# tspooner/rsrl

Hardware: AMD Instinct MI355X
Metric: env-steps/sec (whole node), MountainCar Q-learning Fourier-5 (higher is better)
Workload: dtype f32

## Files before the change

rsrl_amd/_build.py:

```python
import os
import shutil
import subprocess

HERE = os.path.dirname(os.path.abspath(__file__))
CSRC = os.path.join(HERE, "csrc")
LIB_DIR = os.path.join(HERE, "lib")
LIB_PATH = os.path.join(LIB_DIR, "librsrl_hip.so")

HIPCC_FLAGS = ["--offload-arch=gfx950", "-O3", "-std=c++17", "-ffp-contract=off", "-fno-slp-vectorize", "-fPIC",
               "-shared", "-fno-gpu-rdc", "-Wall", "-Wno-unused-function"]


PER_SOURCE_FLAGS = {name: ["-mllvm", "-amdgpu-sched-strategy=" + os.environ.get("RSRL_SCHED_STRATEGY", "max-ilp")]
                    for name in ("train_reg_d0a.hip", "train_reg_d0b.hip", "train_reg_d1.hip", "train_reg_d2.hip")}


ABI_UNITS = ("abi_ctx.hip", "abi_trait.hip", "abi_weights.hip", "abi_train.hip", "abi_group.hip", "kernels_util.hip", "launch_shared.hip")
for _u in ABI_UNITS:
    PER_SOURCE_FLAGS[_u] = ["-mllvm", "-disable-promote-alloca-to-lds"]


def hipcc():
    for cand in (os.environ.get("HIPCC"), shutil.which("hipcc"), "/opt/rocm/bin/hipcc"):
        if cand and os.path.exists(cand):
            return cand
    raise RuntimeError("hipcc not found (need ROCm >= 7.0)")


def sources():
    return [os.path.join(CSRC, f) for f in sorted(os.listdir(CSRC)) if f.endswith(".hip")]


def deps():
    inc = os.path.join(os.path.dirname(HERE), "include", "rsrl_hip.h")
    return [os.path.join(CSRC, f) for f in os.listdir(CSRC)] + [inc, os.path.abspath(__file__), os.path.join(HERE, "_asmfilter.py")]


STAMP_PATH = LIB_PATH + ".sha256"


def source_digest(extra_flags=()):
    import hashlib
    h = hashlib.sha256()
    files = sorted(os.path.join(CSRC, f) for f in os.listdir(CSRC)) + [os.path.join(os.path.dirname(HERE), "include", "rsrl_hip.h")]
    for f in files:
        h.update(os.path.basename(f).encode() + b"\0")
        h.update(open(f, "rb").read())
    h.update(repr((HIPCC_FLAGS, sorted(PER_SOURCE_FLAGS.items()), list(extra_flags), nop_filter_enabled(), NOP_FILTER_SOURCES)).encode())
    h.update(open(os.path.join(HERE, "_asmfilter.py"), "rb").read())
    h.update(hipcc_version().encode())
    return h.hexdigest()


_HIPCC_VERSION = None


def hipcc_version():
    global _HIPCC_VERSION
    if _HIPCC_VERSION is None:
        try:
            _HIPCC_VERSION = subprocess.run([hipcc(), "--version"], capture_output=True, text=True, timeout=60).stdout.strip()
        except Exception:
            _HIPCC_VERSION = ""
    return _HIPCC_VERSION


def is_stale():
# ... 139 lines not shown
```

rsrl_amd/csrc/abi_ctx.hip:

```cpp
#include "ctx.hpp"

thread_local std::string g_last_error;

int fail(int code, const char* fmt, ...) {
    char buf[512];
    va_list ap; va_start(ap, fmt); vsnprintf(buf, sizeof(buf), fmt, ap); va_end(ap);
    g_last_error = buf;
    if (code == RSRL_HIP_EHIP || code == RSRL_HIP_ENOMEM) (void)hipGetLastError();
    return code;
}

static Switches read_switches() {
    Switches sw;
    sw.no_graph = getenv("RSRL_NO_GRAPH") != nullptr;
    sw.no_persist = getenv("RSRL_NO_PERSIST") != nullptr;
    sw.no_trait_defer = getenv("RSRL_NO_TRAIT_DEFER") != nullptr;
    sw.k1_feature_major = getenv("RSRL_K1_FEATURE_MAJOR") != nullptr;
    if (const char* e = getenv("RSRL_K1_QUAD")) sw.k1_quad = e[0] != '0' ? 1 : 0;
    if (const char* e = getenv("RSRL_SPARSE_CHUNK")) { const int v = atoi(e); sw.sparse_chunk = v > 0 && v < 16 ? 16 : v; }
    if (const char* e = getenv("RSRL_PEER_TIMEOUT_MS")) sw.peer_timeout_ms = atol(e);
    if (const char* e = getenv("RSRL_WAVE_PK")) sw.no_wave_pk = e[0] == '0';
    return sw;
}
bool no_coalesce_switch() { return getenv("RSRL_NO_COALESCE") != nullptr; }

static AgentFamily classify(const rsrl_hip_config& cfg, size_t w_elems) {
    using F = AgentFamily;
    const bool fourier = cfg.basis == RSRL_FOURIER, tile = cfg.basis == RSRL_TILE_CODING;
    const bool wave = is_wave(cfg), reg = is_reg_fourier(cfg);
    const int al = cfg.algo;
    if (cfg.domain == RSRL_HIV_TREATMENT) return F::Hiv;
    if (is_ac(al)) return F::AcReg;
    if (is_tdac(al)) return F::TdAcReg;
    if (is_reinforce(al)) return F::ReinforceReg;
    if (is_lstd(al)) return F::LstdReg;
    if (is_tdac_lstd(al)) return F::TdAcLstdReg;
    if (cfg.weight_mode == RSRL_W_SHARED) return fourier ? F::SharedDense : (is_sparse_lambda(cfg) ? F::SharedSparseLambda : F::SharedTile);
    if (wave && is_wave_aux_algo(al)) return F::WaveAux;
    if (is_pred(al)) return tile ? F::TdTile : (reg ? F::TdReg : F::TdGeneric);
    if (al == RSRL_Q_SIGMA) return wave ? F::WaveQSigma : (reg ? F::QSigmaReg : F::QSigmaGeneric);
    if (al == RSRL_GREEDY_GQ) return reg ? F::GqReg : F::GqGeneric;
    if (is_lambda(al)) return tile ? F::LambdaTile : (wave ? F::WaveLambda : (reg ? F::LambdaReg : F::LambdaGeneric));
    if (wave) return F::WaveControl;
    if (reg) return cfg.steps_per_launch == 1 && (uint64_t)w_elems * 4ull < (1ull << 32) ? F::RegStep : F::RegFused;
    return F::Generic;
}
static const char* train_kernel_name(const rsrl_hip_ctx* c) {
    switch (c->family) {
    case AgentFamily::SharedDense: return "k_shared_step";
    case AgentFamily::SharedTile: return "k_shared_ca";
    case AgentFamily::SharedSparseLambda: return "k_sparse_trace_scatter";
    case AgentFamily::WaveAux: return "k_wave_aux";
    case AgentFamily::TdTile: return "k_td_tile";
    case AgentFamily::TdGeneric: return "k_td_mem";
    case AgentFamily::TdReg: return "k_train_td";
    case AgentFamily::WaveQSigma: return "k_wave_qsigma";
    case AgentFamily::QSigmaReg: case AgentFamily::QSigmaGeneric: return "k_train_qsigma";
    case AgentFamily::GqReg: return "k_train_gq";
    case AgentFamily::GqGeneric: return "k_train_gq_mem";
    case AgentFamily::LambdaTile: return "k_lambda_tile";
    case AgentFamily::WaveLambda: return "k_wave_lambda";
    case AgentFamily::LambdaGeneric: return "k_train_lambda_mem";
    case AgentFamily::LambdaReg: return "k_train_lambda";
    case AgentFamily::WaveControl: return c->cfg.weight_dtype == RSRL_W_BF16 && !c->sw.no_wave_pk ? "k_train_wave_pk" : "k_train_wave";
    case AgentFamily::RegStep: return c->w_ls != 1 ? (c->k1_quad ? "k_step_reg_q4" : "k_step_reg_lm") : "k_step_reg";
    case AgentFamily::RegFused: return "k_train_reg";
    case AgentFamily::Generic: return "k_train_mem";
    case AgentFamily::Hiv: return "k_hiv_train";
    case AgentFamily::AcReg: return "k_train_ac";
    case AgentFamily::TdAcReg: return "k_train_tdac";
    case AgentFamily::ReinforceReg: return "k_train_reinforce";
    case AgentFamily::LstdReg: return "k_train_lstd";
    case AgentFamily::TdAcLstdReg: return "k_train_tdac_lstd";
    }
// ... 183 lines not shown
    }
    if (shared && wave) return fail(RSRL_HIP_EINVAL, "shared weights are not available for the order-7 wave family yet");
    if (shared && !tile && !reg)
        return fail(RSRL_HIP_EINVAL, "shared weights need a register-family Fourier order (MountainCar 1-5, CartPole/Acrobot 1) or tile coding");
    if (!f32 && !wave) return fail(RSRL_HIP_EINVAL, "bf16 weights are available for Fourier order 7 on CartPole / Acrobot only");
    if (!model_supported(cfg))
        return fail(RSRL_HIP_EINVAL, "basis %d (order %d / %d tilings) on domain %d has no kernel yet", cfg.basis, cfg.order, cfg.n_tilings, cfg.domain);
    if (is_pred(al)) {
        if (!per_env) return fail(RSRL_HIP_EINVAL, "the prediction agents (TD, TDLambda) need per-learner weights on a Fourier basis or on tile coding");
        if (cfg.policy != RSRL_RANDOM) return fail(RSRL_HIP_EINVAL, "prediction agents have no Q function: the behaviour policy must be RSRL_RANDOM");
    }
    if (al == RSRL_GREEDY_GQ && !per_env) return fail(RSRL_HIP_EINVAL, "GreedyGQ needs per-learner weights");
    if (al == RSRL_Q_SIGMA && !per_env) return fail(RSRL_HIP_EINVAL, "QSigma needs per-learner weights");
    if (is_lambda(al) && !per_env && !is_sparse_lambda(cfg))
        return fail(RSRL_HIP_EINVAL, "the eligibility-trace agents need per-learner weights on a Fourier basis "
                                     "or on tile coding (per-learner tables, or one shared table with sparse per-learner traces)");
    if (esched && !(cfg.policy == RSRL_EPSILON_GREEDY && per_env && cfg.steps_per_launch != 1 && (one_step || (is_lambda(al) && (reg || wave)))))
        return fail(RSRL_HIP_EINVAL, "epsilon_decay (the per-learner epsilon schedule) needs policy = EpsilonGreedy, per-learner weights, steps_per_launch != 1 and "
                                     "a one-step agent or SARSALambda / QLambda on a register-family or order-7 wave-family Fourier basis, or a one-step agent on "
                                     "tile coding / a generic Fourier order");
    return RSRL_HIP_OK;
}

static int create_impl(const rsrl_hip_config* cfg, rsrl_hip_ctx* c) {
    TRY(check_config(*cfg));
    c->cfg = *cfg;
    c->D = kDomainShape[cfg->domain][0]; c->A = kDomainShape[cfg->domain][1];
    c->F = 1;
    for (int i = 0; i < c->D; ++i) c->F *= cfg->basis == RSRL_FOURIER ? cfg->order + 1 : cfg->tiles_per_dim;
    if (cfg->basis == RSRL_TILE_CODING) c->F *= cfg->n_tilings;
    int ndev = 0;
    HIP_TRY(hipGetDeviceCount(&ndev));
    if (ndev < 1) return fail(RSRL_HIP_EHIP, "no HIP device");
    if (cfg->device < 0 || cfg->device >= ndev) return fail(RSRL_HIP_EINVAL, "device %d out of range (%d devices)", cfg->device, ndev);
    HIP_TRY(hipSetDevice(cfg->device));
    { int cus = 0; HIP_TRY(hipDeviceGetAttribute(&cus, hipDeviceAttributeMultiprocessorCount, cfg->device)); if (cus > 0) { c->n_simd = 4 * cus; c->n_cu = cus; } }
    if (cfg->peer_timeout_ms < 0) return fail(RSRL_HIP_EINVAL, "peer_timeout_ms must be >= 0");
    c->sw = read_switches();
    if (cfg->peer_timeout_ms > 0) c->peer_timeout = (uint64_t)cfg->peer_timeout_ms * 100000ull;
    else if (c->sw.peer_timeout_ms > 0) c->peer_timeout = (uint64_t)c->sw.peer_timeout_ms * 100000ull;
    if (cfg->stream) { c->stream = (hipStream_t)cfg->stream; c->own_stream = false; }
    else { HIP_TRY(hipStreamCreateWithFlags(&c->stream, hipStreamNonBlocking)); c->own_stream = true; }
    const int64_t N = cfg->n_envs;
    const bool shared = cfg->weight_mode == RSRL_W_SHARED;
    c->w_stride = shared ? 1 : N;
    c->Aw = (is_pred(cfg->algo) || is_tdac(cfg->algo) || is_lstd(cfg->algo) || is_tdac_lstd(cfg->algo)) ? 1 : c->A;
    c->w_elems = (size_t)c->Aw * c->F * (size_t)(shared ? 1 : N);
    c->family = classify(*cfg, c->w_elems);
    if (c->family == AgentFamily::RegStep && (c->A * c->F) % 4 == 0 && c->F % 4 == 0 && !c->sw.k1_feature_major) {
        c->w_stride = 1;
        c->w_ls = (int64_t)c->A * c->F;
        c->k1_quad = c->A <= 3 && (c->sw.k1_quad >= 0 ? c->sw.k1_quad == 1 : N >= 131072);
    }
    c->train_kernel = train_kernel_name(c);
    c->dw_elems = (size_t)c->Aw * c->F;
    switch (c->family) {
    case AgentFamily::WaveAux: case AgentFamily::WaveQSigma: case AgentFamily::WaveLambda: case AgentFamily::WaveControl: c->n_stat_slots = wave_grid_for(N); break;
    case AgentFamily::TdTile: case AgentFamily::LambdaTile: case AgentFamily::SharedSparseLambda: c->n_stat_slots = (size_t)N; break;
    case AgentFamily::LambdaGeneric: c->n_stat_slots = (size_t)((N + 63) / 64); break;
    case AgentFamily::LstdReg: case AgentFamily::TdAcLstdReg: c->n_stat_slots = (size_t)((N * lstd_group_lanes(c->F) + kBlock - 1) / kBlock); break;
    default: c->n_stat_slots = c->k1_quad ? (size_t)((N + 63) / 64) : grid_for(N); break;
    }
    HIP_TRY(hipMalloc((void**)&c->state, sizeof(float) * c->D * (size_t)N));
    HIP_TRY(hipMalloc((void**)&c->action, sizeof(int32_t) * (size_t)N));
    HIP_TRY(hipMalloc((void**)&c->ep_step, sizeof(uint32_t) * (size_t)N));
    c->w_bytes = c->w_elems * (cfg->weight_dtype == RSRL_W_BF16 ? 2 : 4);
    HIP_TRY(hipMalloc((void**)&c->W, c->w_bytes));
    HIP_TRY(hipMalloc((void**)&c->dW, sizeof(float) * c->dw_elems));
    HIP_TRY(hipMalloc((void**)&c->qcache, sizeof(float) * c->A * (size_t)N));
    if (cfg->domain == RSRL_HIV_TREATMENT) HIP_TRY(hipMalloc((void**)&c->hiv_y, sizeof(double) * 6 * (size_t)N));
    if (c->w_ls != 1 && cfg->weight_dtype == RSRL_W_F32 && cfg->epsilon_decay == 1.0 && trait_lm_available(cfg->domain, cfg->order, cfg->algo)) {
        HIP_TRY(hipMalloc((void**)&c->tq_key, sizeof(float) * c->D * (size_t)N));
        HIP_TRY(hipMalloc((void**)&c->tq_q, sizeof(float) * c->A * (size_t)N));
    }
    if (cfg->algo == RSRL_Q_SIGMA) {
        const size_t nf = (size_t)(c->D + 5) * (size_t)cfg->n_steps * (size_t)N;
        HIP_TRY(hipMalloc((void**)&c->qs_buf, sizeof(float) * nf));
        HIP_TRY(hipMalloc((void**)&c->qs_head, sizeof(uint32_t) * (size_t)N));
        HIP_TRY(hipMalloc((void**)&c->qs_len, sizeof(uint32_t) * (size_t)N));
        HIP_TRY(hipMemsetAsync(c->qs_buf, 0, sizeof(float) * nf, c->stream));
        HIP_TRY(hipMemsetAsync(c->qs_head, 0, sizeof(uint32_t) * (size_t)N, c->stream));
        HIP_TRY(hipMemsetAsync(c->qs_len, 0, sizeof(uint32_t) * (size_t)N, c->stream));
    }
    if (cfg->epsilon_decay != 1.0) {
        HIP_TRY(hipMalloc((void**)&c->eps, sizeof(float) * (size_t)N));
        hipLaunchKernelGGL(k_fill_f32, dim3(grid_for(N)), dim3(kBlock), 0, c->stream, c->eps, N, (float)cfg->epsilon);
        KCHECK();
    }
    if (c->family == AgentFamily::SharedSparseLambda) {
        const int64_t slice = (int64_t)(c->F / cfg->n_tilings) * c->A;
        if (slice > 65536) return fail(RSRL_HIP_EINVAL, "SARSALambda / QLambda over a shared tile table: one tiling's slice (cells * actions = %lld entries) must not "
                                                        "exceed 65 536 (16-bit slice-relative keys between the step and the trace kernel)", (long long)slice);
        HIP_TRY(hipMalloc((void**)&c->sp_keys, sizeof(uint16_t) * (size_t)kSparseCap * (size_t)N));
        HIP_TRY(hipMalloc((void**)&c->sp_vals, sizeof(float) * (size_t)kSparseCap * (size_t)N));
        HIP_TRY(hipMalloc((void**)&c->sp_len, sizeof(uint32_t) * (size_t)cfg->n_tilings * (size_t)N));
        HIP_TRY(hipMemsetAsync(c->sp_len, 0, sizeof(uint32_t) * (size_t)cfg->n_tilings * (size_t)N, c->stream));
        HIP_TRY(hipMemsetAsync(c->sp_keys, 0, sizeof(uint16_t) * (size_t)kSparseCap * (size_t)N, c->stream));
        HIP_TRY(hipMemsetAsync(c->sp_vals, 0, sizeof(float) * (size_t)kSparseCap * (size_t)N, c->stream));
        c->sp_lds = slice * 8 <= 128 * 1024;
        if (c->sp_lds && slice * 8 > 64 * 1024) c->sp_lds = sparse_trace_scatter_allow_lds(cfg->n_tilings, (int)(slice * 8));
    } else if (has_aux(cfg->algo) || is_v_actor_critic(c)) {
        c->z_bytes = (is_v_actor_critic(c) ? (size_t)aux_cols(c) * c->F * (size_t)N : c->w_elems) * 4;
        HIP_TRY(hipMalloc((void**)&c->Z, c->z_bytes));
        HIP_TRY(hipMemsetAsync(c->Z, 0, c->z_bytes, c->stream));
    } else if (c->family == AgentFamily::ReinforceReg) {
        c->z_bytes = c->w_elems * 4;
// ... 289 lines not shown
```

rsrl_amd/csrc/abi_train.hip:

```cpp
#include "ctx.hpp"

RSRL_DEFINE_FX_READER(fx_saturations_train)

int timing_begin(rsrl_hip_ctx* c) {
    if (!c->timing) return RSRL_HIP_OK;
    if (c->events_used == c->events.size()) {
        hipEvent_t a, b;
        HIP_TRY(hipEventCreate(&a)); HIP_TRY(hipEventCreate(&b));
        c->events.emplace_back(a, b);
    }
    HIP_TRY(hipEventRecord(c->events[c->events_used].first, c->stream));
    return RSRL_HIP_OK;
}
int timing_end(rsrl_hip_ctx* c, uint32_t launches) {
    if (!c->timing) return RSRL_HIP_OK;
    HIP_TRY(hipEventRecord(c->events[c->events_used].second, c->stream));
    if (c->event_launches.size() <= c->events_used) c->event_launches.resize(c->events_used + 1);
    c->event_launches[c->events_used] = launches;
    c->events_used++;
    return RSRL_HIP_OK;
}

static inline int fold_in_step(const rsrl_hip_ctx* c) { return !c->multi ? 1 : (c->cfg.exchange == RSRL_EXCHANGE_PEER ? 0 : 1); }
static inline long long* tab_set_of(const rsrl_hip_ctx* c, uint64_t t) { return c->sh_tab + (size_t)kTabRep * c->dw_elems * (size_t)(t % 3u); }
// ... 264 lines not shown
        if (coop_err != hipSuccess) {
            (void)hipGetLastError();
            if (may_fall_back) { c->persist_refused = true; *outcome = PERSIST_FALLBACK; return RSRL_HIP_OK; }
            return fail(RSRL_HIP_ERCCL, "the runtime refused the persistent shared-W grid of rank %d (%u blocks of %d threads on device %d: %s); the other ranks "
                                        "of the group were told it fits -- set RSRL_NO_PERSIST=1 on every rank", c->rank, c->sh_rows, kSharedBlock, c->cfg.device,
                        hipGetErrorString(coop_err));
        }
        c->coop_validated = true;
    }
    KCHECK();
    PersistEntry e;
    e.id = gate.next_id++; e.owner = owner; e.round = round; e.waited = waited;
    HIP_TRY(hipEventCreateWithFlags(&e.ev, hipEventDisableTiming));
    HIP_TRY(hipEventRecord(e.ev, c->stream));
    live.push_back(std::move(e));
    return RSRL_HIP_OK;
}

int launch_agent(rsrl_hip_ctx* c, const Common& k, const BasisGeom& g, uint64_t t, int chunk, DevStats* d_stats, const Transitions* io) {
    const rsrl_hip_config& cf = c->cfg;
    const dim3 grid(grid_for(io ? io->M : k.n_envs)), block(kBlock);
    const bool td_lambda = cf.algo == RSRL_TD_LAMBDA;
    bool ok = true;
    switch (c->family) {
    case AgentFamily::WaveAux: case AgentFamily::WaveQSigma: case AgentFamily::WaveLambda:
        launch_wave_agent(c, k, t, chunk, d_stats, io); break;
    case AgentFamily::TdTile: ok = launch_td_tile(cf.domain, cf.n_tilings, td_lambda, c->stream, k, g, make_td(c), t, chunk, d_stats, io); break;
    case AgentFamily::TdGeneric: ok = launch_td_model(cf, grid, block, c->stream, k, make_td(c), g, td_lambda, t, chunk, d_stats, io); break;
    case AgentFamily::TdReg: ok = launch_td(cf.domain, cf.order, td_lambda, grid, block, c->stream, k, make_td(c), t, chunk, d_stats, io); break;
    case AgentFamily::QSigmaReg: ok = launch_qsigma(cf.domain, cf.order, grid, block, c->stream, k, make_qs(c), g, t, chunk, d_stats, io); break;
    case AgentFamily::QSigmaGeneric: ok = launch_qsigma_model(cf, grid, block, c->stream, k, make_qs(c), g, t, chunk, d_stats, io); break;
    case AgentFamily::GqReg: ok = launch_gq(cf.domain, cf.order, cf.policy, grid, block, c->stream, k, make_gq(c), t, chunk, d_stats, io); break;
    case AgentFamily::GqGeneric: ok = launch_gq_model(cf, grid, block, c->stream, k, make_gq(c), g, t, chunk, d_stats, io); break;
    case AgentFamily::LambdaTile: ok = launch_lambda_tile(cf.domain, cf.n_tilings, c->stream, k, g, make_lambda(c), t, chunk, d_stats, io); break;
    case AgentFamily::LambdaGeneric: ok = launch_lambda_model(cf, grid, block, c->stream, k, make_lambda(c), g, t, chunk, d_stats, io); break;
    case AgentFamily::LambdaReg: ok = launch_lambda(cf.domain, cf.order, cf.algo, cf.policy, grid, block, c->stream, k, make_lambda(c), t, chunk, d_stats, io); break;
    case AgentFamily::WaveControl:
        for_wave(c, [&](auto tag) {
            using T = decltype(tag); using WT = typename T::wt;
            const dim3 wg(wave_grid_for(k.n_envs));
            if constexpr (WaveIO<WT>::kBf16) {
                if (!c->sw.no_wave_pk) {
                    if (k.eps) hipLaunchKernelGGL((k_train_wave_pk<T::domain, true>), wg, block, 0, c->stream, k, (WT*)c->W, t, chunk, d_stats);
                    else hipLaunchKernelGGL((k_train_wave_pk<T::domain>), wg, block, 0, c->stream, k, (WT*)c->W, t, chunk, d_stats);
                    return;
                }
            }
            if (k.eps) hipLaunchKernelGGL((k_train_wave<T::domain, WT, true>), wg, block, 0, c->stream, k, (WT*)c->W, t, chunk, d_stats);
            else hipLaunchKernelGGL((k_train_wave<T::domain, WT>), wg, block, 0, c->stream, k, (WT*)c->W, t, chunk, d_stats);
        });
        break;
    case AgentFamily::RegStep: return enqueue_k1_step(c, k, d_stats, t, nullptr);
    case AgentFamily::RegFused:
        switch (cf.domain) {
        case 0: ok = launch_train_reg_d0(cf.order, cf.algo, cf.policy, grid, block, c->stream, k, t, chunk, d_stats); break;
        case 1: ok = launch_train_reg_d1(cf.order, cf.algo, cf.policy, grid, block, c->stream, k, t, chunk, d_stats); break;
        default: ok = launch_train_reg_d2(cf.order, cf.algo, cf.policy, grid, block, c->stream, k, t, chunk, d_stats); break;
        }
        break;
    case AgentFamily::Generic:
        ok = for_model(c, [&](auto tag) {
            using M = typename decltype(tag)::type;
            hipLaunchKernelGGL((k_train_mem<M>), grid, block, 0, c->stream, k, g, t, chunk, d_stats);
        });
        break;
    case AgentFamily::Hiv:
        if (io) launch_hiv_handle(c->stream, k, g, *io, t);
        else launch_hiv_train(c->stream, k, g, c->hiv_y, t, chunk, d_stats);
        break;
    case AgentFamily::AcReg:
        ok = launch_ac(cf.domain, cf.order, cf.algo == RSRL_Q_ACTOR_CRITIC ? AC_CRITIC_Q : AC_CRITIC_ADVANTAGE, grid, block, c->stream, k, c->Z, t, chunk, d_stats, io);
        break;
    case AgentFamily::TdAcReg: ok = launch_tdac(cf.domain, cf.order, grid, block, c->stream, k, c->Z, t, chunk, d_stats, io); break;
    case AgentFamily::LstdReg: ok = launch_lstd(cf.domain, cf.order, cf.algo == RSRL_ILSTD, c->stream, k, make_lstd(c), t, chunk, d_stats, io); break;
    case AgentFamily::TdAcLstdReg: ok = launch_tdac_lstd(cf.domain, cf.order, c->stream, k, make_tdac_lstd(c), t, chunk, d_stats, io); break;
    case AgentFamily::ReinforceReg:
        ok = !io && launch_reinforce(cf.domain, cf.order, cf.algo == RSRL_BASELINE_REINFORCE, grid, block, c->stream, k, make_reinforce(c), t, chunk, d_stats, nullptr);
        break;
    default: ok = false; break;
    }
    if (!ok) return NO_MODEL(c);
    KCHECK();
    return RSRL_HIP_OK;
}

int train_now(rsrl_hip_ctx* c, int64_t n_steps, rsrl_hip_stats* stats_out) {
    HIP_TRY(hipSetDevice(c->cfg.device));
    c->tq_valid = false;
    DevStats* d_stats = stats_out ? c->d_stats : nullptr;
    if (d_stats) HIP_TRY(hipMemsetAsync(c->d_stats, 0, sizeof(DevStats) * c->n_stat_slots, c->stream));
    Common k = make_common(c);
    const BasisGeom g = make_geom(c);
    const bool shared = c->cfg.weight_mode == RSRL_W_SHARED;
    const bool dense = c->family == AgentFamily::SharedDense;
    const int64_t spl = shared ? 1 : fuse_depth(c);
    const bool stream_k1 = c->family == AgentFamily::RegStep;
    const bool graph_ok = (stream_k1 || shared) && c->own_stream && !stats_out && !c->sw.no_graph;
    bool t_dev_set = false;
    int64_t done = 0;
    bool persist = shared && n_steps > 0 && persist_ok(c);
    if (persist) {
        for (int64_t left = n_steps; left > 0;) {
            const int64_t chunk = left < (int64_t)1 << 30 ? left : (int64_t)1 << 30;
            TRY(timing_begin(c));
            int outcome = PERSIST_LAUNCHED;
            TRY(persist_launch(c, k, g, chunk, d_stats, !c->multi && left == n_steps, &outcome));
// ... 165 lines not shown
```

rsrl_amd/csrc/ctx.hpp:

```cpp
#pragma once
#include <hip/hip_runtime.h>
#include <rccl/rccl.h>

#include <cmath>
#include <cstdarg>
#include <cstdio>
#include <cstring>
#include <unistd.h>
#include <dlfcn.h>
#include <map>
#include <mutex>
#include <string>
#include <vector>

#include "../../include/rsrl_hip.h"
#pragma GCC visibility push(hidden)
#define RSRL_API_BEGIN _Pragma("GCC visibility push(default)") extern "C" {
#define RSRL_API_END } _Pragma("GCC visibility pop")
#include "launch.hpp"
#include "models.hpp"
#include "model_list.hpp"
#include "kernels_wave.hpp"
#include "kernels_lambda.hpp"
#include "kernels_gq.hpp"
// ... 45 lines not shown
int fail(int code, const char* fmt, ...);
#define HIP_TRY(expr)                                                                              \
    do {                                                                                           \
        hipError_t _e = (expr);                                                                    \
        if (_e != hipSuccess)                                                                      \
            return fail(_e == hipErrorOutOfMemory ? RSRL_HIP_ENOMEM : RSRL_HIP_EHIP, "%s failed: %s (%s:%d)", \
                        #expr, hipGetErrorString(_e), __FILE__, __LINE__);                         \
    } while (0)
#define CHECK_CTX(ctx) do { if (!(ctx)) return fail(RSRL_HIP_EINVAL, "null ctx"); } while (0)

struct Scratch { void* p = nullptr; size_t cap = 0; };

enum class AgentFamily : uint8_t {
    SharedDense,
    SharedTile,
    SharedSparseLambda,
    WaveAux,
    TdTile,
    TdGeneric,
    TdReg,
    WaveQSigma,
    QSigmaReg,
    QSigmaGeneric,
    GqReg,
    GqGeneric,
    LambdaTile,
    WaveLambda,
    LambdaGeneric,
    LambdaReg,
    WaveControl,
    RegStep,
    RegFused,
    Generic,
    Hiv,
    AcReg,
    TdAcReg,
    ReinforceReg,
    LstdReg,
    TdAcLstdReg,
};
static inline bool is_wave_family(AgentFamily f) {
    return f == AgentFamily::WaveAux || f == AgentFamily::WaveQSigma || f == AgentFamily::WaveLambda || f == AgentFamily::WaveControl;
}

struct Switches {
    bool no_graph = false;
    bool no_persist = false;
    bool no_trait_defer = false;
    bool k1_feature_major = false;
    int k1_quad = -1;
    int sparse_chunk = 0;
    long peer_timeout_ms = 0;
    bool no_wave_pk = false;
};

struct rsrl_hip_ctx {
    rsrl_hip_config cfg{};
    AgentFamily family = AgentFamily::Generic;
    const char* train_kernel = "";
    Switches sw;
    int D = 0, A = 0, F = 0;
    hipStream_t stream = nullptr;
    bool own_stream = false;
    float* state = nullptr; int32_t* action = nullptr; uint32_t* ep_step = nullptr;
    float* W = nullptr; float* dW = nullptr;
    int Aw = 0;
    long long* dW_rep = nullptr; int n_rep = 1;
    long long* sh_tab = nullptr;
    long long* h_fx = nullptr;
    bool tile_slice = false;
    uint16_t* sc_keys = nullptr;
    float* sc_terms = nullptr;
    uint64_t sh_tab_t = 0;
    float* W2 = nullptr;
    int sh_par = 0;
    unsigned sh_rows = 0;
    float* qcache = nullptr;
    float* qs_buf = nullptr; uint32_t* qs_head = nullptr; uint32_t* qs_len = nullptr;
    float* eps = nullptr;
    uint16_t* sp_keys = nullptr; float* sp_vals = nullptr; uint32_t* sp_len = nullptr;
    bool sp_lds = false;
    float* Z = nullptr;
    float* Zb = nullptr;
    float* ret_g = nullptr;
    double* hiv_y = nullptr;
    double* lstd_theta = nullptr;
    double* lstd_mat = nullptr;
    double* lstd_mu = nullptr;
    bool q_valid = false;
    float* tq_key = nullptr;
    float* tq_q = nullptr;
    bool tq_valid = false;
    struct TraitPend { int stage = 0; const int32_t* act = nullptr; float* from = nullptr; float* to = nullptr; float* rew = nullptr;
                       uint8_t* term = nullptr; float* td = nullptr; uint64_t t_handle = 0; } tp;
    uint8_t* flags = nullptr;
    size_t w_elems = 0; size_t dw_elems = 0; size_t w_bytes = 0; size_t z_bytes = 0;
    int64_t w_stride = 0;
    int64_t w_ls = 1;
    DevStats* d_stats = nullptr; DevStats* h_stats = nullptr;
    size_t n_stat_slots = 0;
    bool k1_quad = false;
    uint64_t t = 0;
    int64_t pending = 0;
    uint64_t api_calls = 0;
    uint64_t rollout_calls = 0;
    Scratch scratch[8];
    bool timing = false;
    std::vector<std::pair<hipEvent_t, hipEvent_t>> events;
    std::vector<uint32_t> event_launches;
    size_t events_used = 0;
    uint64_t* d_t = nullptr;
    DynParams* d_dyn = nullptr;
    DynParams dyn_uploaded{};
    bool dyn_valid = false;
    hipGraph_t step_graph = nullptr;
    hipGraphExec_t step_graph_exec = nullptr;
    Common step_graph_key{};
    int step_graph_kind = 0;
    const char* kernel_name = "";
    ncclComm_t comm = nullptr;
    int n_simd = 1024;
    int world_size = 1, rank = 0;
    bool multi = false;
    uint2* peer_recv = nullptr; size_t peer_recv_bytes = 0; int peer_world = 0;
    std::vector<void*> peer_ptrs; std::vector<char> peer_opened;
    uint2** d_peer_ptrs = nullptr;
    uint32_t* d_peer_err = nullptr;
    uint64_t peer_seq = 0;
    uint64_t peer_timeout = 400000000ull;
    size_t peer_old_bytes = 0;
    unsigned long long* px_A = nullptr; unsigned long long* px_B = nullptr; bool px_B_owned = false;
    unsigned long long** d_px_Bptrs = nullptr;
    uint64_t px_seq = 0;
    int n_cu = 256;
    int persist_occ = -1;
    bool group_persist = false;
    int peer_share = 1;
    bool coop_allowed = true;
    bool coop_validated = false;
    bool persist_refused = false;
    uint64_t group_token = 0;
    bool st_rccl_group = false;
};

static Common make_common(const rsrl_hip_ctx* c) {
    Common k{};
    k.n_envs = c->cfg.n_envs; k.env_offset = c->cfg.env_offset; k.seed = c->cfg.seed;
    k.pol.kind = c->cfg.policy;
    double v = c->cfg.epsilon * 16777216.0;
    k.pol.eps_thr = v <= 0.0 ? 0u : (v >= 16777216.0 ? 16777216u : (uint32_t)v);
    k.pol.eps = (float)c->cfg.epsilon; k.pol.tau = (float)c->cfg.tau;
    if (c->cfg.agent_policy < 0) { k.apol = k.pol; k.apol_same = 1; }
    else {
        k.apol.kind = c->cfg.agent_policy;
// ... 281 lines not shown
```

rsrl_amd/csrc/launch.hpp:

```cpp
#pragma once
#include "kernels_reg.hpp"
#include "kernels_reg_q4.hpp"

namespace rsrl {

bool launch_train_reg_d0(int order, int algo, int policy, dim3 grid, dim3 block, hipStream_t st,
                         const Common& k, uint64_t t, int chunk, DevStats* stats, const uint64_t* t_dev = nullptr);
bool launch_train_reg_d1(int order, int algo, int policy, dim3 grid, dim3 block, hipStream_t st,
                         const Common& k, uint64_t t, int chunk, DevStats* stats, const uint64_t* t_dev = nullptr);
bool launch_train_reg_d2(int order, int algo, int policy, dim3 grid, dim3 block, hipStream_t st,
                         const Common& k, uint64_t t, int chunk, DevStats* stats, const uint64_t* t_dev = nullptr);


struct Transitions {
    const float* from = nullptr; const int32_t* act = nullptr; const float* rew = nullptr; const float* to = nullptr; const uint8_t* term = nullptr;
    int64_t M = 0; float* td_out = nullptr;
};
static inline Transitions transitions_or_none(const Transitions* io) { return io ? *io : Transitions{}; }

struct LambdaParams;
struct BasisGeom;
bool launch_lambda(int domain, int order, int algo, int policy, dim3 grid, dim3 block, hipStream_t st, const Common& k, const LambdaParams& lp,
                   uint64_t t, int chunk, DevStats* stats, const Transitions* io);
bool launch_lambda_tile(int domain, int n_tilings, hipStream_t st, const Common& k, const BasisGeom& g, const LambdaParams& lp, uint64_t t, int chunk,
                        DevStats* stats, const Transitions* io);

struct TdParams;
bool launch_td_tile(int domain, int n_tilings, bool lambda, hipStream_t st, const Common& k, const BasisGeom& g, const TdParams& tp, uint64_t t, int chunk,
                    DevStats* stats, const Transitions* io);
bool launch_v_tile(int domain, int n_tilings, hipStream_t st, const Common& k, const BasisGeom& g, const float* states, int64_t M, float* out);

struct GqParams;
bool launch_gq(int domain, int order, int policy, dim3 grid, dim3 block, hipStream_t st, const Common& k, const GqParams& gp, uint64_t t, int chunk,
               DevStats* stats, const Transitions* io);

bool launch_ac(int domain, int order, int critic, dim3 grid, dim3 block, hipStream_t st, const Common& k, float* theta, uint64_t t, int chunk,
               DevStats* stats, const Transitions* io);
bool launch_tdac(int domain, int order, dim3 grid, dim3 block, hipStream_t st, const Common& k, float* theta, uint64_t t, int chunk, DevStats* stats,
                 const Transitions* io);
struct ReinforceState {
    float* theta = nullptr;
    float* theta_b = nullptr;
    float* g = nullptr;
};
struct ReinforceBatch {
    const float* states = nullptr; const int32_t* act = nullptr; const float* rew = nullptr; const uint32_t* len = nullptr; int64_t T = 0;
    float* ret_out = nullptr;
};
bool launch_reinforce(int domain, int order, bool baseline, dim3 grid, dim3 block, hipStream_t st, const Common& k, const ReinforceState& rs, uint64_t t,
                      int chunk, DevStats* stats, const ReinforceBatch* io);
void launch_reinforce_restart(hipStream_t st, const ReinforceState& rs, int64_t N, int64_t FA, const uint8_t* mask);

struct LstdState {
    double* theta = nullptr;
    double* mat = nullptr;
    double* mu = nullptr;
    double gamma = 0.0, alpha = 0.0;
    int n_updates = 0;
};
static inline int lstd_group_lanes(int F) { return F <= 4 ? 4 : (F <= 16 ? 16 : (F <= 32 ? 32 : 64)); }
bool launch_lstd(int domain, int order, bool incremental, hipStream_t st, const Common& k, const LstdState& ls, uint64_t t, int chunk, DevStats* stats,
                 const Transitions* io);
bool launch_lstd_v(int domain, int order, hipStream_t st, const double* theta, const float* states, int64_t M, float* out);
void launch_lstd_sample(int domain, hipStream_t st, const Common& k, uint64_t t, uint32_t blk, int32_t* out);
// ... 71 lines not shown
```

Before: 71.44 billion.

## Add producer-consumer warp-specialized kernel for Fourier-5 MountainCar Q-learning

```diff
diff --git a/rsrl_amd/_build.py b/rsrl_amd/_build.py
--- a/rsrl_amd/_build.py
+++ b/rsrl_amd/_build.py
@@ -12,7 +12,7 @@
 
 
 PER_SOURCE_FLAGS = {name: ["-mllvm", "-amdgpu-sched-strategy=" + os.environ.get("RSRL_SCHED_STRATEGY", "max-ilp")]
-                    for name in ("train_reg_d0a.hip", "train_reg_d0b.hip", "train_reg_d1.hip", "train_reg_d2.hip")}
+                    for name in ("train_reg_d0a.hip", "train_reg_d0b.hip", "train_reg_d1.hip", "train_reg_d2.hip", "train_reg_pw.hip")}
 
 
 ABI_UNITS = ("abi_ctx.hip", "abi_trait.hip", "abi_weights.hip", "abi_train.hip", "abi_group.hip", "kernels_util.hip", "launch_shared.hip")
diff --git a/rsrl_amd/csrc/abi_ctx.hip b/rsrl_amd/csrc/abi_ctx.hip
--- a/rsrl_amd/csrc/abi_ctx.hip
+++ b/rsrl_amd/csrc/abi_ctx.hip
@@ -20,6 +20,7 @@
     if (const char* e = getenv("RSRL_SPARSE_CHUNK")) { const int v = atoi(e); sw.sparse_chunk = v > 0 && v < 16 ? 16 : v; }
     if (const char* e = getenv("RSRL_PEER_TIMEOUT_MS")) sw.peer_timeout_ms = atol(e);
     if (const char* e = getenv("RSRL_WAVE_PK")) sw.no_wave_pk = e[0] == '0';
+    if (const char* e = getenv("RSRL_REG_PRODUCER")) sw.no_reg_producer = e[0] == '0';
     return sw;
 }
 bool no_coalesce_switch() { return getenv("RSRL_NO_COALESCE") != nullptr; }
@@ -309,6 +310,11 @@
         c->w_ls = (int64_t)c->A * c->F;
         c->k1_quad = c->A <= 3 && (c->sw.k1_quad >= 0 ? c->sw.k1_quad == 1 : N >= 131072);
     }
+    if (c->family == AgentFamily::RegFused && !c->sw.no_reg_producer && cfg->epsilon_decay == 1.0 && N <= (int64_t)kBlock * c->n_cu) {
+        int lds = 0;
+        HIP_TRY(hipDeviceGetAttribute(&lds, hipDeviceAttributeMaxSharedMemoryPerBlock, cfg->device));
+        c->reg_producer = train_reg_pw_serves(cfg->domain, cfg->order, cfg->algo, lds);
+    }
     c->train_kernel = train_kernel_name(c);
     c->dw_elems = (size_t)c->Aw * c->F;
     switch (c->family) {
diff --git a/rsrl_amd/csrc/abi_train.hip b/rsrl_amd/csrc/abi_train.hip
--- a/rsrl_amd/csrc/abi_train.hip
+++ b/rsrl_amd/csrc/abi_train.hip
@@ -340,6 +340,7 @@
         break;
     case AgentFamily::RegStep: return enqueue_k1_step(c, k, d_stats, t, nullptr);
     case AgentFamily::RegFused:
+        if (c->reg_producer && !k.eps) { ok = launch_train_reg_pw(cf.algo, cf.policy, grid, c->stream, k, t, chunk, d_stats); break; }
         switch (cf.domain) {
         case 0: ok = launch_train_reg_d0(cf.order, cf.algo, cf.policy, grid, block, c->stream, k, t, chunk, d_stats); break;
         case 1: ok = launch_train_reg_d1(cf.order, cf.algo, cf.policy, grid, block, c->stream, k, t, chunk, d_stats); break;
diff --git a/rsrl_amd/csrc/ctx.hpp b/rsrl_amd/csrc/ctx.hpp
--- a/rsrl_amd/csrc/ctx.hpp
+++ b/rsrl_amd/csrc/ctx.hpp
@@ -121,6 +121,7 @@
     int sparse_chunk = 0;
     long peer_timeout_ms = 0;
     bool no_wave_pk = false;
+    bool no_reg_producer = false;
 };
 
 struct rsrl_hip_ctx {
@@ -169,6 +170,7 @@
     DevStats* d_stats = nullptr; DevStats* h_stats = nullptr;
     size_t n_stat_slots = 0;
     bool k1_quad = false;
+    bool reg_producer = false;
     uint64_t t = 0;
     int64_t pending = 0;
     uint64_t api_calls = 0;
diff --git a/rsrl_amd/csrc/kernels_reg_pw.hpp b/rsrl_amd/csrc/kernels_reg_pw.hpp
--- /dev/null
+++ b/rsrl_amd/csrc/kernels_reg_pw.hpp
@@ -0,0 +1,257 @@
+#pragma once
+
+#include "kernels_reg.hpp"
+
+namespace rsrl {
+namespace pw {
+
+constexpr int kConsumerWaves = kBlock / 64;
+constexpr int kBlockPw = 2 * kBlock;
+constexpr int kRingPairs = 8;
+typedef uint32_t u4v __attribute__((ext_vector_type(4)));
+
+constexpr size_t lds_bytes(bool inner) { return (size_t)kConsumerWaves * 2 * kRingPairs * (inner ? 2 : 1) * 64 * sizeof(u4v) + 512; }
+
+constexpr int kGetregSimdId = 4 | (4 << 6) | (1 << 11);
+
+__device__ __forceinline__ void block_stats_accumulate(DevStats* __restrict__ stats, bool consumer, int cw, unsigned long long n_ep,
+                                                       unsigned long long n_trunc, unsigned long long sum_len, double sum_abs, double sum_r) {
+    __shared__ unsigned long long sh_u[3][kConsumerWaves];
+    __shared__ double sh_d[2][kConsumerWaves];
+    n_ep = wave_sum(n_ep); n_trunc = wave_sum(n_trunc); sum_len = wave_sum(sum_len);
+    sum_abs = wave_sum(sum_abs); sum_r = wave_sum(sum_r);
+    if (consumer && (threadIdx.x & 63) == 0) {
+        sh_u[0][cw] = n_ep; sh_u[1][cw] = n_trunc; sh_u[2][cw] = sum_len;
+        sh_d[0][cw] = sum_abs; sh_d[1][cw] = sum_r;
+    }
+    __syncthreads();
+    if (threadIdx.x == 0) {
+        DevStats acc = stats[blockIdx.x];
+        for (int w = 0; w < kConsumerWaves; ++w) {
+            acc.episodes += sh_u[0][w]; acc.episodes_truncated += sh_u[1][w]; acc.sum_episode_steps += sh_u[2][w];
+            acc.sum_abs_td_error += sh_d[0][w]; acc.sum_reward += sh_d[1][w];
+        }
+        stats[blockIdx.x] = acc;
+    }
+}
+
+template <int DOMAIN, int ORDER, int ALGO, int POLICY, bool STATS = true>
+__global__ __launch_bounds__(kBlockPw, 1) void k_train_reg(Common c, uint64_t t0, int n_steps, DevStats* __restrict__ stats) {
+    using Dom = Domain<DOMAIN>;
+    using Bas = FourierReg<DOMAIN, ORDER>;
+    constexpr int D = Dom::D, A = Dom::A, F = Bas::F;
+    constexpr bool INNER = ALGO == ALG_SARSA;
+    constexpr int NS = INNER ? 2 : 1, H = kRingPairs;
+    static_assert((H & (H - 1)) == 0, "ring slots are taken modulo 2H by a mask");
+    __shared__ u4v ring[kConsumerWaves][2 * H][NS][64];
+    __shared__ int claim[4];
+    static_assert(sizeof(ring) + 512 == lds_bytes(INNER), "lds_bytes() is what the launcher checks against the device");
+
+    const int lane = (int)(threadIdx.x & 63);
+    const int wave = __builtin_amdgcn_readfirstlane((int)(threadIdx.x >> 6));
+    if (threadIdx.x < 4) claim[threadIdx.x] = 0;
+    __syncthreads();
+    const int simd = (int)(__builtin_amdgcn_s_getreg(kGetregSimdId) & 3u);
+    int slot = 0;
+    if (lane == 0) slot = atomicAdd(&claim[simd], 1);
+    __syncthreads();
+    const int paired = __builtin_amdgcn_readfirstlane((claim[0] == 2 && claim[1] == 2 && claim[2] == 2 && claim[3] == 2) ? 1 : 0);
+    slot = __builtin_amdgcn_readfirstlane(slot);
+    const bool consumer = paired ? slot == 0 : wave < kConsumerWaves;
+    const int cw = paired ? simd : (wave & (kConsumerWaves - 1));
+
+    const int64_t N = c.n_envs;
+    const int64_t blk0 = (int64_t)blockIdx.x * kBlock;
+    const int64_t i = blk0 + cw * 64 + lane;
+    const uint64_t th0 = t0 >> 1;
+    const int NB = n_steps > 0 ? (int)(((t0 + (uint64_t)n_steps - 1) >> 1) - th0) + 1 : 0;
+    const int G = (NB + H - 1) / H;
+
+    uint32_t n_ep = 0, n_trunc = 0, sum_len = 0;
+    double sum_abs = 0.0, sum_r = 0.0;
+
+    if (!consumer) {
+        const uint32_t gid = (uint32_t)(c.env_offset + i);
+        for (int g = 0; g < G; ++g) {
+            const int b1 = min((g + 1) * H, NB);
+            for (int b = g * H; b < b1; ++b) {
+                const U4 p = draw_block(c.seed, gid, th0 + (uint64_t)b, BLK_STEP);
+                ring[cw][b & (2 * H - 1)][0][lane] = u4v{p.x, p.y, p.z, p.w};
+                if constexpr (INNER) {
+                    const U4 q = draw_block(c.seed, gid, th0 + (uint64_t)b, BLK_INNER);
+                    ring[cw][b & (2 * H - 1)][NS - 1][lane] = u4v{q.x, q.y, q.z, q.w};
+                }
+            }
+            __syncthreads();
+        }
+    } else {
+        const bool valid = i < N;
+        const int64_t il = valid ? i : N - 1;
+        char* __restrict__ const wblk = reinterpret_cast<char*>(c.W + blk0 * c.w_ls);
+        const uint32_t wlane = (uint32_t)(il - blk0) * (uint32_t)c.w_ls * 4u;
+        const int64_t wrow = c.w_stride * 4;
+
+        PolicyParams pol = c.pol; pol.kind = POLICY;
+        AlgoParams alg = c.alg; alg.kind = ALGO;
+        const uint32_t cap = c.max_episode_steps;
+        float s[D];
+#pragma unroll
+        for (int d = 0; d < D; ++d) s[d] = c.state[(int64_t)d * N + il];
+        int a = c.action[il];
+        uint32_t ep = c.ep_step[il];
+        const uint32_t ep_start = ep;
+        constexpr bool PK = (RSRL_PK != 0) && (F % 4 == 0);
+        using Phi = PhiBuf<F, PK>;
+        WBuf<A, F, PK> w;
+#pragma unroll
+        for (int b = 0; b < A; ++b)
+#pragma unroll
+            for (int f = 0; f < F; ++f) w.put(b, f, row_load(wblk + (int64_t)(b * F + f) * wrow, wlane));
+
+        static_assert(A <= 3, "QCarry holds up to 3 actions");
+        Phi phi_a, phi_b;
+        QCarry q_s;
+        { float ph[F]; Bas::project(s, ph); phi_a.set(ph); }
+        {
+            float q0[A];
+            if (c.q_valid) {
+#pragma unroll
+                for (int b = 0; b < A; ++b) q0[b] = c.qcache[(int64_t)b * N + il];
+            } else {
+                w.q(phi_a, q0);
+            }
+            q_s.set<A>(q0);
+        }
+        typename Dom::Pre pre_s = Dom::pre(s);
+        float facc_abs = 0.0f, facc_r = 0.0f;
+        __builtin_amdgcn_s_waitcnt(0x0070);
+
+        auto one_step = [&](const Phi& phi_s, Phi& phi_n, const U4& x, const U4& xin) {
+            float ns[D];
+#pragma unroll
+            for (int d = 0; d < D; ++d) ns[d] = s[d];
+            float r;
+            const bool term = Dom::step(ns, a, r, pre_s);
+            ep += 1;
+            const bool trunc = !term && cap > 0 && ep >= cap;
+            if (term) Dom::reset(ns);
+            pre_s = Dom::pre(ns);
+            float q_n[A];
+            { float ph[F]; Bas::project(ns, ph); phi_n.set(ph); }
+            w.q(phi_n, q_n);
+            static_assert(A <= 3, "ActionMask covers three actions");
+            const ActionMask am(a);
+            const float qsa = A > 2 ? bitsel(am.m2, q_s.v2, bitsel(am.m1, q_s.v1, q_s.v0)) : bitsel(am.m1, q_s.v1, q_s.v0);
+            const float q_s_all[3] = {q_s.v0, q_s.v1, q_s.v2};
+            float e;
+            float delta;
+            if constexpr (ALGO == ALG_PAL) {
+                float qs_arr[A];
+#pragma unroll
+                for (int b = 0; b < A; ++b) qs_arr[b] = q_s_all[b];
+                delta = td_error_pal<A>(alg, qs_arr, q_n, a, r, term, e);
+            } else {
+                delta = td_error_ap<A, ALGO>(alg, pol, c, qsa, q_n, r, term, xin, e);
+            }
+            const float scale = alg.lr * e;
+            {
+                float sb[A];
+#pragma unroll
+                for (int b = 0; b < A; ++b) sb[b] = and_mask(am.of(b), scale);
+                w.axpy(sb, phi_s);
+            }
+            {
+                const float dot = Phi::dot(phi_s, phi_n);
+#pragma unroll
+                for (int b = 0; b < A; ++b) q_n[b] = bitsel(am.of(b), fmaf(scale, dot, q_n[b]), q_n[b]);
+            }
+            int na = policy_sample<A, true>(pol, q_n, x);
+            if constexpr (STATS) {
+                facc_abs += fabsf(delta);
+                facc_r += r;
+                n_ep += term ? 1u : 0u;
+            }
+            ep = term ? 0u : ep;
+            if (__builtin_expect(trunc, 0)) {
+                if constexpr (STATS) { n_ep += 1; n_trunc += 1; }
+                ep = 0;
+                Dom::reset(ns);
+                pre_s = Dom::pre(ns);
+                { float ph[F]; Bas::project(ns, ph); phi_n.set(ph); }
+                w.q(phi_n, q_n);
+                na = policy_sample<A, true>(pol, q_n, x);
+            }
+#pragma unroll
+            for (int d = 0; d < D; ++d) s[d] = ns[d];
+            q_s.set<A>(q_n);
+            a = na;
+        };
+
+        auto ring_read = [&](int b, int st) {
+            const u4v v = ring[cw][b & (2 * H - 1)][st][lane];
+            return U4{v.x, v.y, v.z, v.w};
+        };
+        const U4 zero4 = U4{0, 0, 0, 0};
+        const bool lead = (t0 & 1u) && n_steps > 0;
+        const bool trail = n_steps > 0 && ((t0 + (uint64_t)n_steps) & 1u);
+        const int b_end = NB - (trail ? 1 : 0);
+
+        __builtin_amdgcn_s_setprio(1);
+        int b = 0;
+        if (G > 0) __syncthreads();
+        if (lead) {
+            const U4 p = ring_read(0, 0), pin = INNER ? ring_read(0, NS - 1) : zero4;
+            one_step(phi_a, phi_b, half_block(p, true), half_block(pin, true));
+            const Phi tmp = phi_a; phi_a = phi_b; phi_b = tmp;
+            b = 1;
+        }
+        for (int g = 0; g < G; ++g) {
+            if (g > 0) __syncthreads();
+            const int ge = min((g + 1) * H, b_end);
+            if (b < ge) {
+                U4 nx = ring_read(b, 0), nxin = INNER ? ring_read(b, NS - 1) : zero4;
+                for (; b < ge; ++b) {
+                    const U4 p = nx, pin = nxin;
+                    const int bn = min(b + 1, ge - 1);
+                    nx = ring_read(bn, 0);
+                    if constexpr (INNER) nxin = ring_read(bn, NS - 1);
+                    one_step(phi_a, phi_b, half_block(p, false), half_block(pin, false));
+                    one_step(phi_b, phi_a, half_block(p, true), half_block(pin, true));
+                }
+            }
+        }
+        if (trail) {
+            const U4 p = ring_read(NB - 1, 0), pin = INNER ? ring_read(NB - 1, NS - 1) : zero4;
+            one_step(phi_a, phi_b, half_block(p, false), half_block(pin, false));
+        }
+        __builtin_amdgcn_s_setprio(0);
+
+        if (valid) {
+            sum_abs = (double)facc_abs; sum_r = (double)facc_r;
+            sum_len = (uint32_t)n_steps + ep_start - ep;
+#pragma unroll
+            for (int d = 0; d < D; ++d) c.state[(int64_t)d * N + i] = s[d];
+            c.action[i] = a;
+            c.ep_step[i] = ep;
+            c.qcache[i] = q_s.v0;
+            if constexpr (A > 1) c.qcache[N + i] = q_s.v1;
+            if constexpr (A > 2) c.qcache[2 * N + i] = q_s.v2;
+            char* wblk_e = wblk;
+            int64_t wrow_e = wrow;
+            asm volatile("" : "+s"(wblk_e), "+s"(wrow_e));
+#pragma unroll
+            for (int bb = 0; bb < A; ++bb)
+#pragma unroll
+                for (int f = 0; f < F; ++f) row_store(wblk_e + (int64_t)(bb * F + f) * wrow_e, wlane, w.get(bb, f));
+        } else {
+            n_ep = 0; n_trunc = 0;
+        }
+    }
+
+    if constexpr (STATS) {
+        if (stats) block_stats_accumulate(stats, consumer, cw, n_ep, n_trunc, sum_len, sum_abs, sum_r);
+    }
+}
+
+}
+}
diff --git a/rsrl_amd/csrc/launch.hpp b/rsrl_amd/csrc/launch.hpp
--- a/rsrl_amd/csrc/launch.hpp
+++ b/rsrl_amd/csrc/launch.hpp
@@ -10,6 +10,9 @@
                          const Common& k, uint64_t t, int chunk, DevStats* stats, const uint64_t* t_dev = nullptr);
 bool launch_train_reg_d2(int order, int algo, int policy, dim3 grid, dim3 block, hipStream_t st,
                          const Common& k, uint64_t t, int chunk, DevStats* stats, const uint64_t* t_dev = nullptr);
+
+bool train_reg_pw_serves(int domain, int order, int algo, int lds_limit_bytes);
+bool launch_train_reg_pw(int algo, int policy, dim3 grid, hipStream_t st, const Common& k, uint64_t t, int chunk, DevStats* stats);
 
 
 struct Transitions {
diff --git a/rsrl_amd/csrc/train_reg_pw.hip b/rsrl_amd/csrc/train_reg_pw.hip
--- /dev/null
+++ b/rsrl_amd/csrc/train_reg_pw.hip
@@ -0,0 +1,22 @@
+#include "launch.hpp"
+#include "kernels_reg_pw.hpp"
+namespace rsrl {
+bool train_reg_pw_serves(int domain, int order, int algo, int lds_limit_bytes) {
+    if (domain != 0 || order != 5) return false;
+    if (algo != 0 && algo != 1 && algo != 2 && algo != 5) return false;
+    return (size_t)(lds_limit_bytes > 0 ? lds_limit_bytes : 0) >= pw::lds_bytes(algo == ALG_SARSA);
+}
+#define RSRL_PW_CASE(AL, PO)                                                                                              \
+    if (algo == AL && policy == PO) {                                                                                     \
+        if (!stats)                     \
+            hipLaunchKernelGGL((pw::k_train_reg<0, 5, AL, PO, false>), grid, dim3(pw::kBlockPw), 0, st, k, t, chunk, stats); \
+        else                                                                                                              \
+            hipLaunchKernelGGL((pw::k_train_reg<0, 5, AL, PO>), grid, dim3(pw::kBlockPw), 0, st, k, t, chunk, stats);     \
+        return true;                                                                                                      \
+    }
+#define RSRL_PW_POLICIES(AL) RSRL_PW_CASE(AL, 0) RSRL_PW_CASE(AL, 1) RSRL_PW_CASE(AL, 2) RSRL_PW_CASE(AL, 3)
+bool launch_train_reg_pw(int algo, int policy, dim3 grid, hipStream_t st, const Common& k, uint64_t t, int chunk, DevStats* stats) {
+    RSRL_PW_POLICIES(0) RSRL_PW_POLICIES(1) RSRL_PW_POLICIES(2) RSRL_PW_POLICIES(5)
+    return false;
+}
+}
```

Measured after the change: 74.39 billion (median of 6 runs). +4.1%, better.
